# LukasHaas/PIGEON

Measured on AMD Instinct MI355X. Metric: images/sec end-to-end (ViT+head+refine), 4x336x336, higher is better.
Workload: dtype f16

## Files before the change

### pigeon_amd/csrc/attention.hip

```cpp
#include "attention_common.h"

constexpr int ATT8_NQB = 2, ATT8_WAVES = 4, ATT8_WPS = 3;

template <typename T, int NQB>
__device__ __forceinline__ void att8_exp_pack(const f32x4 (&S)[4][NQB], typename T::v8 (&pf)[NQB][2]) {
#pragma unroll
    for (int qb = 0; qb < NQB; ++qb) {
#pragma unroll
        for (int j = 0; j < 2; ++j) {
            u32x4 pw;
#pragma unroll
            for (int h = 0; h < 2; ++h)
#pragma unroll
                for (int w = 0; w < 2; ++w) {
                    const f32x4& sv = S[2 * j + h][qb];
                    pw[2 * h + w] = T::pack2(__builtin_amdgcn_exp2f(sv[2 * w]), __builtin_amdgcn_exp2f(sv[2 * w + 1]));
                }
            pf[qb][j] = __builtin_bit_cast(typename T::v8, pw);
        }
    }
}

template <typename T, int NQB>
__device__ __forceinline__ void att8_softmax(f32x4 (&S)[4][NQB], f32x4 (&O)[4][NQB], f32x4 (&negm)[NQB], typename T::v8 (&pf)[NQB][2],
                                             bool first, f32x4 (&L)[NQB]) {
    float tmax[NQB];
    bool over = false;
#pragma unroll
    for (int qb = 0; qb < NQB; ++qb) {
        float t = max3f(S[0][qb][0], S[0][qb][1], S[0][qb][2]);
        t = max3f(t, S[0][qb][3], S[1][qb][0]);
        t = max3f(t, S[1][qb][1], S[1][qb][2]);
        t = max3f(t, S[1][qb][3], S[2][qb][0]);
        t = max3f(t, S[2][qb][1], S[2][qb][2]);
        t = max3f(t, S[2][qb][3], S[3][qb][0]);
        t = max3f(t, S[3][qb][1], S[3][qb][2]);
        t = __builtin_fmaxf(t, S[3][qb][3]);
        t = __builtin_fmaxf(t, __shfl_xor(t, 16, 64));
        t = __builtin_fmaxf(t, __shfl_xor(t, 32, 64));
        tmax[qb] = t;
        over = over || t > ATT_LAZY_THR;
    }
    if (first || __builtin_amdgcn_ballot_w64(over) != 0) {
#pragma unroll
        for (int qb = 0; qb < NQB; ++qb) {
            const float delta = (first || tmax[qb] > ATT_LAZY_THR) ? tmax[qb] : 0.f;
            const float alpha = first ? 1.f : __builtin_amdgcn_exp2f(-delta);
            const float nm = negm[qb][0] - delta;
            negm[qb] = f32x4{nm, nm, nm, nm};
#pragma unroll
            for (int kb = 0; kb < 4; ++kb) S[kb][qb] -= delta;
#pragma unroll
            for (int db = 0; db < 4; ++db) O[db][qb] *= alpha;
            L[qb] *= alpha;
        }
    }
    att8_exp_pack<T, NQB>(S, pf);
}

__device__ __forceinline__ void att8_dma(__amdgpu_buffer_rsrc_t r, char* dst, int wave, const int* dvo, int ndma, int waves, int t) {
#pragma unroll
    for (int i = 0; i < ndma; ++i)
        __builtin_amdgcn_raw_ptr_buffer_load_lds(r, (att_lds_void*)(dst + (wave + waves * i) * 8 * K_ROWB), 16, dvo[i],
                                                 t * (ATT_KT * QKV_LD * 2), 0, 0);
}
__device__ __forceinline__ void att8_load_v(u32x4 (&vf)[4][2], const char* vs, const int (&vb)[4]) {
    const uint32_t vs_lds = (uint32_t)(uintptr_t)(__attribute__((address_space(3))) const char*)vs;
    __builtin_amdgcn_sched_barrier(0);
#define ATT8_TR(db, j)                                                                                        \
    {                                                                                                         \
        const u32x2 lo = att_tr_read<((j) * 32) * K_ROWB>(vs_lds + vb[db]);                                   \
        const u32x2 hi = att_tr_read<((j) * 32 + 16) * K_ROWB>(vs_lds + vb[db]);                              \
        vf[db][j] = u32x4{lo[0], lo[1], hi[0], hi[1]};                                                        \
    }
    ATT8_TR(0, 0) ATT8_TR(1, 0) ATT8_TR(2, 0) ATT8_TR(3, 0) ATT8_TR(0, 1) ATT8_TR(1, 1) ATT8_TR(2, 1) ATT8_TR(3, 1)
#undef ATT8_TR
    __builtin_amdgcn_sched_barrier(0);
}
__device__ __forceinline__ void att8_wait_v(u32x4 (&vf)[4][2]) {
    asm volatile("s_waitcnt lgkmcnt(0)"
                 : "+v"(vf[0][0]), "+v"(vf[1][0]), "+v"(vf[2][0]), "+v"(vf[3][0]), "+v"(vf[0][1]), "+v"(vf[1][1]),
                   "+v"(vf[2][1]), "+v"(vf[3][1])
                 :: "memory");
}

template <typename T>
__global__ __launch_bounds__(ATT8_WAVES * 64, ATT8_WPS) void attention8_kernel(const uint16_t* __restrict__ qkv, uint16_t* __restrict__ out) {
    constexpr int NQB = ATT8_NQB, WAVES = ATT8_WAVES;
    constexpr int QB = NQB * WAVES * 16;
    static_assert(QB * ATT_NQB >= VIT_TOKENS, "the blocks of an (image, head) cover every query");
    static_assert(VIT_TOKENS == 9 * ATT_KT + 1, "key tail assumes 577 tokens");
    __shared__ __attribute__((aligned(16))) char smem[4 * K_TILE_BYTES];
    char* ks0 = smem;
    char* vs0 = smem + 2 * K_TILE_BYTES;
    const int tid = threadIdx.x, lane = tid & 63;
    const int wave = __builtin_amdgcn_readfirstlane(tid >> 6);
    const int r16 = lane & 15, g4 = lane >> 4;
    const int bid = blockIdx.x;
    const int xcd = bid & 7, slot = bid >> 3;
    const int qblk = slot % ATT_NQB;
    const int pair = (slot / ATT_NQB) * 8 + xcd;
    const int img = pair >> 4, head = pair & 15;
    const int64_t base = (int64_t)img * VIT_TOKENS;
    const int q_first = qblk * QB + wave * (NQB * 16);
    const bool wave_active = q_first < VIT_TOKENS;

    typename T::v8 qf[NQB][2];
#pragma unroll
    for (int qb = 0; qb < NQB; ++qb) {
        int qr = q_first + 16 * qb + r16;
        qr = qr < VIT_TOKENS ? qr : VIT_TOKENS - 1;
#pragma unroll
        for (int ks = 0; ks < 2; ++ks)
            qf[qb][ks] = *(const typename T::v8*)(qkv + (base + qr) * QKV_LD + head * 64 + ks * 32 + g4 * 8);
    }
    f32x4 O[4][NQB], negm[NQB];
    f32x4 L[NQB];
    const u32x4 ones_rows = r16 == 0 ? u32x4{AttOnes<T>::v, AttOnes<T>::v, AttOnes<T>::v, AttOnes<T>::v} : u32x4{0u, 0u, 0u, 0u};
#pragma unroll
    for (int qb = 0; qb < NQB; ++qb) {
        negm[qb] = f32x4{0.f, 0.f, 0.f, 0.f};
        L[qb] = f32x4{0.f, 0.f, 0.f, 0.f};
#pragma unroll
        for (int db = 0; db < 4; ++db) O[db][qb] = f32x4{0.f, 0.f, 0.f, 0.f};
    }
    int kx[2];
#pragma unroll
    for (int ks = 0; ks < 2; ++ks) kx[ks] = r16 * K_ROWB + (((4 * ks + g4) ^ ((r16 >> 1) & 7)) << 4);
    int vb[4];
    {
        const int f = (2 * g4 + (r16 >> 3)) & 3;
#pragma unroll
        for (int db = 0; db < 4; ++db) vb[db] = (4 * g4 + (r16 >> 2)) * K_ROWB + ((db ^ f) << 5) + ((r16 & 3) << 3);
    }
    __amdgpu_buffer_rsrc_t rk = __builtin_amdgcn_make_buffer_rsrc(
        const_cast<uint16_t*>(qkv + base * QKV_LD + 1024 + head * 64), (short)0, (int)(VIT_TOKENS * QKV_LD * 2), 0x00020000);
    __amdgpu_buffer_rsrc_t rv = __builtin_amdgcn_make_buffer_rsrc(
        const_cast<uint16_t*>(qkv + base * QKV_LD + 2048 + head * 64), (short)0, (int)(VIT_TOKENS * QKV_LD * 2), 0x00020000);
    constexpr int NDMA = 8 / WAVES;
    const bool stager = wave < WAVES;
    int dvo_k[NDMA], dvo_v[NDMA];
#pragma unroll
    for (int i = 0; i < NDMA; ++i) {
        const int row = ((wave & (WAVES - 1)) + WAVES * i) * 8 + (lane >> 3);
        dvo_k[i] = row * (QKV_LD * 2) + (((lane & 7) ^ ((row >> 1) & 7)) << 4);
        dvo_v[i] = row * (QKV_LD * 2) + (((lane & 7) ^ (((row >> 1) & 3) << 1)) << 4);
    }
    constexpr int NFULL = 9;

    if (stager) {
        att8_dma(rk, ks0, wave, dvo_k, NDMA, WAVES, 0);
        att8_dma(rv, vs0, wave, dvo_v, NDMA, WAVES, 0);
    }
    asm volatile("s_waitcnt vmcnt(0)" ::: "memory");
    __syncthreads();
    for (int t = 0; t < NFULL; ++t) {
        const int cur = t & 1;
        if (t + 1 < NFULL && stager) {
            att8_dma(rk, ks0 + (cur ^ 1) * K_TILE_BYTES, wave, dvo_k, NDMA, WAVES, t + 1);
            att8_dma(rv, vs0 + (cur ^ 1) * K_TILE_BYTES, wave, dvo_v, NDMA, WAVES, t + 1);
        }
        const char* ks = ks0 + cur * K_TILE_BYTES;
        const char* vs = vs0 + cur * K_TILE_BYTES;
        if (wave_active) {
            f32x4 S[4][NQB];
            typename T::v8 pf[NQB][2];
            {
                typename T::v8 kf[4][2];
#pragma unroll
                for (int kb = 0; kb < 4; ++kb)
#pragma unroll
                    for (int ks_ = 0; ks_ < 2; ++ks_) kf[kb][ks_] = *(const typename T::v8*)(ks + kb * 16 * K_ROWB + kx[ks_]);
                __builtin_amdgcn_sched_barrier(0);
#pragma unroll
                for (int ks_ = 0; ks_ < 2; ++ks_)
#pragma unroll
                    for (int kb = 0; kb < 4; ++kb)
#pragma unroll
                        for (int qb = 0; qb < NQB; ++qb)
                            S[kb][qb] = T::mfma16(kf[kb][ks_], qf[qb][ks_], ks_ == 0 ? negm[qb] : S[kb][qb]);
            }
            u32x4 vf[4][2];
            att8_load_v(vf, vs, vb);
            att8_softmax<T, NQB>(S, O, negm, pf, t == 0, L);
            att8_wait_v(vf);
#pragma unroll
            for (int j = 0; j < 2; ++j)
#pragma unroll
                for (int db = 0; db < 4; ++db)
#pragma unroll
                    for (int qb = 0; qb < NQB; ++qb)
                        O[db][qb] = T::mfma16(__builtin_bit_cast(typename T::v8, vf[db][j]), pf[qb][j], O[db][qb]);
#pragma unroll
            for (int j = 0; j < 2; ++j)
#pragma unroll
                for (int qb = 0; qb < NQB; ++qb)
                    L[qb] = T::mfma16(__builtin_bit_cast(typename T::v8, ones_rows), pf[qb][j], L[qb]);
        }
        asm volatile("s_waitcnt vmcnt(0)" ::: "memory");
        __syncthreads();
    }
    if (!wave_active) return;

    const uint16_t* krow = qkv + (base + (VIT_TOKENS - 1)) * QKV_LD + 1024 + head * 64;
    const uint16_t* vrow = krow + 1024;
    u32x4 kq[2];
#pragma unroll
    for (int ks = 0; ks < 2; ++ks) kq[ks] = *(const u32x4*)(krow + ks * 32 + g4 * 8);
    u32x2 vv[4];
#pragma unroll
    for (int db = 0; db < 4; ++db) vv[db] = *(const u32x2*)(vrow + db * 16 + g4 * 4);
#pragma unroll
    for (int qb = 0; qb < NQB; ++qb) {
        float sp = 0.f;
#pragma unroll
        for (int ks = 0; ks < 2; ++ks) {
            const u32x4 qq = __builtin_bit_cast(u32x4, qf[qb][ks]);
#pragma unroll
            for (int w = 0; w < 4; ++w) sp = T::dot2(qq[w], kq[ks][w], sp);
        }
        sp += __shfl_xor(sp, 16, 64);
        const float sc = sp + __shfl_xor(sp, 32, 64);
        const float m = -negm[qb][0];
        const float m_new = fmaxf(m, sc);
        const float alpha = __builtin_amdgcn_exp2f(m - m_new);
        const float pk = __builtin_amdgcn_exp2f(sc - m_new);
        const float l = L[qb][0] * alpha + (g4 == 0 ? pk : 0.f);
#pragma unroll
        for (int db = 0; db < 4; ++db)
#pragma unroll
            for (int e = 0; e < 4; ++e) {
                const uint16_t hb = (uint16_t)(vv[db][e >> 1] >> (16 * (e & 1)));
                O[db][qb][e] = fmaf(pk, T::val(hb), O[db][qb][e] * alpha);
            }
        float lt = l + __shfl_xor(l, 16, 64);
        lt += __shfl_xor(lt, 32, 64);
        const float inv = 1.0f / lt;
        const int qrow = q_first + 16 * qb + r16;
        if (qrow < VIT_TOKENS) {
            uint16_t* orow = out + (base + qrow) * VIT_HIDDEN + head * 64;
#pragma unroll
            for (int db = 0; db < 4; ++db) {
                u32x2 pk2;
                pk2[0] = pack16x2<T>(O[db][qb][0] * inv, O[db][qb][1] * inv);
                pk2[1] = pack16x2<T>(O[db][qb][2] * inv, O[db][qb][3] * inv);
                *(u32x2*)(orow + db * 16 + g4 * 4) = pk2;
            }
        }
    }
}


int pg_attention_launch(int dtype, const void* qkv, void* out, int n_images, hipStream_t s) {
    if (n_images <= 0) return PG_OK;
    if (dtype != PG_DTYPE_F16 && dtype != PG_DTYPE_BF16) { pg_set_error("attention: dtype must be PG_DTYPE_F16 or PG_DTYPE_BF16"); return PG_EINVAL; }
    const int pairs = n_images * VIT_HEADS;
    const dim3 grid(pairs * ATT_NQB), block(ATT8_WAVES * 64);
    if (dtype == PG_DTYPE_F16) hipLaunchKernelGGL(attention8_kernel<T_F16>, grid, block, 0, s, (const uint16_t*)qkv, (uint16_t*)out);
    else hipLaunchKernelGGL(attention8_kernel<T_BF16>, grid, block, 0, s, (const uint16_t*)qkv, (uint16_t*)out);
    return pg_check_launch("attention");
}
```

### pigeon_amd/csrc/attention_common.h

```cpp
#pragma once
#include "common.h"
#include "pigeon_internal.h"

#define ATT_KT 64
#define ATT_QB 128
#define ATT_NQB 5
#define ATT_NT 10
#define K_ROWB 128
#define VT_STRIDE 136
#define K_TILE_BYTES (ATT_KT * K_ROWB)
#define VT_TILE_BYTES (64 * VT_STRIDE)
#define QKV_LD 3072
#define ATT_LAZY_THR 8.0f

typedef __attribute__((address_space(3))) void att_lds_void;

template <int OFF>
__device__ __forceinline__ u32x2 att_tr_read(uint32_t addr) {
    u32x2 r;
    asm volatile("ds_read_b64_tr_b16 %0, %1 offset:%2" : "=v"(r) : "v"(addr), "n"(OFF));
    return r;
}
template <typename T> struct AttOnes;
template <> struct AttOnes<T_F16> { static constexpr uint32_t v = 0x3C003C00u; };
template <> struct AttOnes<T_BF16> { static constexpr uint32_t v = 0x3F803F80u; };
```

Measured before the change: 2501.

## Skip max tracking in attention tiles unless row sums grow past a threshold

After the first key tile, the attention loop now exponentiates scores against the existing running max and uses the rowsum MFMA to detect whether any row's sum grew by more than a trigger amount. Only when a wave sees such growth does it restore L, recompute QK, reload V and run the full online-softmax rescale path. The aim is to drop the per-tile max/rescale work in the common case, at the cost of an extra rowsum check and a full recompute in the rare case, plus a possible looser bound on fp16 overflow. Optional probe counters are added behind a compile flag.

```diff
diff --git a/pigeon_amd/csrc/attention.hip b/pigeon_amd/csrc/attention.hip
--- a/pigeon_amd/csrc/attention.hip
+++ b/pigeon_amd/csrc/attention.hip
@@ -83,6 +83,41 @@
                    "+v"(vf[2][1]), "+v"(vf[3][1])
                  :: "memory");
 }
+
+template <typename T, int NQB>
+__device__ __forceinline__ void att8_qk(f32x4 (&S)[4][NQB], const char* ks, const int (&kx)[2], const typename T::v8 (&qf)[NQB][2],
+                                        const f32x4 (&negm)[NQB]) {
+    typename T::v8 kf[4][2];
+#pragma unroll
+    for (int kb = 0; kb < 4; ++kb)
+#pragma unroll
+        for (int ks_ = 0; ks_ < 2; ++ks_) kf[kb][ks_] = *(const typename T::v8*)(ks + kb * 16 * K_ROWB + kx[ks_]);
+    __builtin_amdgcn_sched_barrier(0);
+#pragma unroll
+    for (int ks_ = 0; ks_ < 2; ++ks_)
+#pragma unroll
+        for (int kb = 0; kb < 4; ++kb)
+#pragma unroll
+            for (int qb = 0; qb < NQB; ++qb)
+                S[kb][qb] = T::mfma16(kf[kb][ks_], qf[qb][ks_], ks_ == 0 ? negm[qb] : S[kb][qb]);
+}
+template <typename T, int NQB>
+__device__ __forceinline__ void att8_rowsum(f32x4 (&L)[NQB], const u32x4& ones_rows, const typename T::v8 (&pf)[NQB][2]) {
+#pragma unroll
+    for (int j = 0; j < 2; ++j)
+#pragma unroll
+        for (int qb = 0; qb < NQB; ++qb)
+            L[qb] = T::mfma16(__builtin_bit_cast(typename T::v8, ones_rows), pf[qb][j], L[qb]);
+}
+
+#ifdef PIGEON_PROBES
+__device__ unsigned long long pg_dbg_att_rare[2][9];
+extern "C" int pg_dbg_att_rare_read(unsigned long long* out18, int reset) {
+    if (hipMemcpyFromSymbol(out18, HIP_SYMBOL(pg_dbg_att_rare), sizeof(unsigned long long) * 18) != hipSuccess) return PG_EHIP;
+    if (reset) { unsigned long long z[18] = {0}; if (hipMemcpyToSymbol(HIP_SYMBOL(pg_dbg_att_rare), z, sizeof(z)) != hipSuccess) return PG_EHIP; }
+    return PG_OK;
+}
+#endif
 
 template <typename T>
 __global__ __launch_bounds__(ATT8_WAVES * 64, ATT8_WPS) void attention8_kernel(const uint16_t* __restrict__ qkv, uint16_t* __restrict__ out) {
@@ -165,24 +200,38 @@
         if (wave_active) {
             f32x4 S[4][NQB];
             typename T::v8 pf[NQB][2];
-            {
-                typename T::v8 kf[4][2];
-#pragma unroll
-                for (int kb = 0; kb < 4; ++kb)
-#pragma unroll
-                    for (int ks_ = 0; ks_ < 2; ++ks_) kf[kb][ks_] = *(const typename T::v8*)(ks + kb * 16 * K_ROWB + kx[ks_]);
-                __builtin_amdgcn_sched_barrier(0);
-#pragma unroll
-                for (int ks_ = 0; ks_ < 2; ++ks_)
-#pragma unroll
-                    for (int kb = 0; kb < 4; ++kb)
-#pragma unroll
-                        for (int qb = 0; qb < NQB; ++qb)
-                            S[kb][qb] = T::mfma16(kf[kb][ks_], qf[qb][ks_], ks_ == 0 ? negm[qb] : S[kb][qb]);
-            }
+            att8_qk<T, NQB>(S, ks, kx, qf, negm);
             u32x4 vf[4][2];
             att8_load_v(vf, vs, vb);
-            att8_softmax<T, NQB>(S, O, negm, pf, t == 0, L);
+            if (t == 0) {
+                att8_softmax<T, NQB>(S, O, negm, pf, true, L);
+                att8_rowsum<T, NQB>(L, ones_rows, pf);
+            } else {
+                att8_exp_pack<T, NQB>(S, pf);
+                float lsave[NQB];
+#pragma unroll
+                for (int qb = 0; qb < NQB; ++qb) lsave[qb] = L[qb][0];
+                att8_rowsum<T, NQB>(L, ones_rows, pf);
+                bool grew = false;
+#pragma unroll
+                for (int qb = 0; qb < NQB; ++qb) grew = grew || L[qb][0] - lsave[qb] >= ATT_ROWSUM_TRIG;
+#ifdef PIGEON_PROBES
+                if (lane == 0) atomicAdd(&pg_dbg_att_rare[1][t], 1ull);
+#endif
+                if (__builtin_amdgcn_ballot_w64(grew) != 0) {
+                    att8_wait_v(vf);
+#ifdef PIGEON_PROBES
+                    if (lane == 0) atomicAdd(&pg_dbg_att_rare[0][t], 1ull);
+#endif
+#pragma unroll
+                    for (int qb = 0; qb < NQB; ++qb) L[qb] = f32x4{lsave[qb], 0.f, 0.f, 0.f};
+                    att8_qk<T, NQB>(S, ks, kx, qf, negm);
+                    att8_load_v(vf, vs, vb);
+                    att8_softmax<T, NQB>(S, O, negm, pf, false, L);
+                    att8_rowsum<T, NQB>(L, ones_rows, pf);
+                }
+            }
+            __builtin_amdgcn_sched_barrier(0);
             att8_wait_v(vf);
 #pragma unroll
             for (int j = 0; j < 2; ++j)
@@ -191,11 +240,6 @@
 #pragma unroll
                     for (int qb = 0; qb < NQB; ++qb)
                         O[db][qb] = T::mfma16(__builtin_bit_cast(typename T::v8, vf[db][j]), pf[qb][j], O[db][qb]);
-#pragma unroll
-            for (int j = 0; j < 2; ++j)
-#pragma unroll
-                for (int qb = 0; qb < NQB; ++qb)
-                    L[qb] = T::mfma16(__builtin_bit_cast(typename T::v8, ones_rows), pf[qb][j], L[qb]);
         }
         asm volatile("s_waitcnt vmcnt(0)" ::: "memory");
         __syncthreads();
diff --git a/pigeon_amd/csrc/attention_common.h b/pigeon_amd/csrc/attention_common.h
--- a/pigeon_amd/csrc/attention_common.h
+++ b/pigeon_amd/csrc/attention_common.h
@@ -12,6 +12,7 @@
 #define VT_TILE_BYTES (64 * VT_STRIDE)
 #define QKV_LD 3072
 #define ATT_LAZY_THR 8.0f
+#define ATT_ROWSUM_TRIG 128.0f
 
 typedef __attribute__((address_space(3))) void att_lds_void;
 
```

Result: no change. 2517, median of 6 (+0.6%).
